# paplorinc/jtokkit

Measured on AMD Instinct MI355X. Metric: input MB/s encoded (cl100k_base), HBM-resident input and output, bit-exact vs CPU oracle, higher is better.
Workload: dtype int32; 1 GPU; cl100k_base, 1M mixed UTF-8 docs (emoji + CJK, ~4 KB each); docs=1000000, bytes=4099377688, docs_per_gpu=1000000, bytes_per_gpu=4099377688, encode=encode() incl. the special-token check

## Files before the change

jtokkit_amd/csrc/jtk_abi.cpp:

```cpp
#include <hip/hip_runtime.h>

#include <algorithm>
#include <cstdio>
#include <cstdlib>
#include <cstring>
#include <new>
#include <string>
#include <vector>
#include <thread>
#include <chrono>

#include "../../include/jtokkit_amd.h"
#include "jtk_chunk_rules.h"
#include "jtk_chunk_prefer_rules.h"
#include "jtk_compact_rules.h"
#include "jtk_decode_rows_rules.h"
#include "jtk_kernels.h"
#include "jtk_maxtok_rules.h"
#include "jtk_tables.h"

namespace {

thread_local std::string g_err;

// ... 198 lines not shown
    if (sp.empty() || n_bytes <= 0) return;
    bool first[256] = {false};
    for (auto& x : sp) if (!x.first.empty()) first[(uint8_t)x.first[0]] = true;
    const size_t slice = (size_t)1 << 22;
    const size_t n_slices = ((size_t)n_bytes + slice - 1) / slice;
    host_slices(n_slices, [&](int, size_t lo, size_t hi) {
        const int64_t b0 = (int64_t)(lo * slice), b1 = std::min<int64_t>(n_bytes, (int64_t)(hi * slice));
        for (int fb = 0; fb < 256; fb++) {
            if (!first[fb]) continue;
            const uint8_t* p = utf8 + b0;
            const uint8_t* const endp = utf8 + b1;
            while (p < endp) {
                p = (const uint8_t*)memchr(p, fb, (size_t)(endp - p));
                if (!p) break;
                const int64_t pos = p - utf8;
                for (auto& x : sp) {
                    const std::string& lit = x.first;
                    if (lit.empty() || (uint8_t)lit[0] != (uint8_t)fb || pos + (int64_t)lit.size() > n_bytes) continue;
                    if (memcmp(p, lit.data(), lit.size()) != 0) continue;
                    const int64_t d = (std::upper_bound(doc_off, doc_off + n_docs + 1, pos) - doc_off) - 1;
                    if (d >= 0 && d < n_docs && pos + (int64_t)lit.size() <= doc_off[d + 1]) flag[(size_t)d] = 1;
                }
                p++;
            }
        }
    });
}



extern "C" {

const char* jtk_version(void) { return "jtokkit_amd 0.1 (gfx950; Unicode " JTK_UNICODE_VERSION " class tables)"; }
const char* jtk_last_error(void) { return g_err.c_str(); }

int jtk_device_count(void) {
    int n = 0;
    hipError_t e = hipGetDeviceCount(&n);
    if (e != hipSuccess) return fail(JTK_ERR_NO_DEVICE, std::string("hipGetDeviceCount: ") + hipGetErrorString(e));
    return n;
}

int jtk_encoding_create(const char* name, int pattern_kind, const uint8_t* tiktoken, size_t tiktoken_len,
                        const char* const* special_literals, const int32_t* special_ids, int n_specials,
                        int device, jtk_encoding** out) {
    if (!out) return fail(JTK_ERR_INVALID_ARGUMENT, "out is NULL");
    *out = nullptr;
    if (!tiktoken || n_specials < 0 || (n_specials > 0 && (!special_literals || !special_ids)))
        return fail(JTK_ERR_INVALID_ARGUMENT, "bad arguments");
    if (n_specials > JTK_MAX_SPECIALS) return fail(JTK_ERR_INVALID_ARGUMENT, "too many special tokens");
    for (int i = 0; i < n_specials; i++) {
        const size_t l = strlen(special_literals[i]);
        if (l < 1 || l > JTK_SPECIAL_MAXLEN)
            return fail(JTK_ERR_INVALID_ARGUMENT, "special-token literals must be 1..65535 bytes long");
        if (special_ids[i] < 0 || special_ids[i] > JTK_MAX_SPECIAL_ID)
            return fail(JTK_ERR_INVALID_ARGUMENT, "special-token id out of range");
    }
    jtk_encoding* enc = new (std::nothrow) jtk_encoding();
    if (!enc) return fail(JTK_ERR_OUT_OF_MEMORY, "out of host memory");
    std::string err;
    int rc = jtk_build_tables(name, pattern_kind, tiktoken, tiktoken_len, special_literals, special_ids, n_specials,
                              enc->host, err);
    if (rc != JTK_OK) { delete enc; return fail(rc, err); }
    enc->tok_len.assign((size_t)enc->host.max_id + 1 + (size_t)enc->host.n_missing, 1);
    {
        int64_t top = (int64_t)enc->host.max_id + (int64_t)enc->host.n_missing;
        for (auto& sp : enc->host.specials) top = std::max<int64_t>(top, sp.second);
        enc->hb = jtk_compact_hb(top);
    }
    for (size_t i = 0; i <= (size_t)enc->host.max_id; i++) enc->tok_len[i] = (uint32_t)enc->host.id_to_bytes[i].size();

    int ndev = 0;
    if (hipGetDeviceCount(&ndev) != hipSuccess || ndev <= 0) {
        delete enc;
        return fail(JTK_ERR_NO_DEVICE, "no HIP device: jtokkit_amd has no CPU path");
    }
    if (device < 0 || device >= ndev) { delete enc; return fail(JTK_ERR_INVALID_ARGUMENT, "device index out of range"); }
    enc->device = device;
    auto cleanup = [&]() { enc->uc1.release(); enc->uc2.release(); enc->uclds.release(); enc->splittab.release(); enc->brank.release(); enc->pairs.release(); enc->tok8.release(); enc->tok16.release(); enc->bprank.release(); enc->bpbits.release(); enc->bpcum.release(); enc->bpranks.release(); enc->pairin.release(); enc->dec_off.release(); enc->dec_blob.release(); enc->longtok.release(); enc->longblob.release(); enc->specials.release(); enc->bnd.release(); delete enc; };
#define ENC_TRY(expr) do { hipError_t e_ = (expr); if (e_ != hipSuccess) { cleanup(); return fail(JTK_ERR_HIP, std::string(#expr) + ": " + hipGetErrorString(e_)); } } while (0)
    ENC_TRY(hipSetDevice(device));
    const size_t tok8_bytes = (enc->host.tok8.size() * sizeof(JtkTok8Slot) + 31) & ~(size_t)31;
    std::vector<uint8_t> uc_image;
    if (sizeof(jtk_uc_stage1_init) <= JTK_UC_LDS_STAGE1 && JTK_UC_LDS_STAGE1 + sizeof(jtk_uc_stage2_init) <= (size_t)JTK_UC_LDS_UNITS * 16) {
        uc_image.assign((size_t)JTK_UC_LDS_UNITS * 16, 0);
        memcpy(uc_image.data(), jtk_uc_stage1_init, sizeof(jtk_uc_stage1_init));
        memcpy(uc_image.data() + JTK_UC_LDS_STAGE1, jtk_uc_stage2_init, sizeof(jtk_uc_stage2_init));
    }
    if (enc->uc1.ensure(sizeof(jtk_uc_stage1_init)) || enc->uc2.ensure(sizeof(jtk_uc_stage2_init)) ||
        enc->uclds.ensure(uc_image.size() + 16) || enc->splittab.ensure(256 * sizeof(JtkCode4)) ||
        enc->brank.ensure(256 * 4) || enc->pairs.ensure(enc->host.pair_buckets.size() * sizeof(JtkPairBucket)) ||
        enc->tok8.ensure(tok8_bytes + enc->host.tok16.size() * sizeof(JtkTok16Slot) + 32) ||
        enc->bprank.ensure(65536 * 4) ||
        enc->bpbits.ensure(1024 * 8) || enc->bpcum.ensure(1024 * 2) || enc->bpranks.ensure(JTK_BP_MAX * 4) || enc->pairin.ensure(2048 * 4)) { cleanup(); return JTK_ERR_OUT_OF_MEMORY; }
    ENC_TRY(hipMemcpy(enc->uc1.p, jtk_uc_stage1_init, sizeof(jtk_uc_stage1_init), hipMemcpyHostToDevice));
    ENC_TRY(hipMemcpy(enc->uc2.p, jtk_uc_stage2_init, sizeof(jtk_uc_stage2_init), hipMemcpyHostToDevice));
    if (!uc_image.empty()) ENC_TRY(hipMemcpy(enc->uclds.p, uc_image.data(), uc_image.size(), hipMemcpyHostToDevice));
    ENC_TRY(hipMemcpy(enc->brank.p, enc->host.byte_rank, 256 * 4, hipMemcpyHostToDevice));
    ENC_TRY(hipMemcpy(enc->pairs.p, enc->host.pair_buckets.data(), enc->host.pair_buckets.size() * sizeof(JtkPairBucket), hipMemcpyHostToDevice));
    ENC_TRY(hipMemcpy(enc->tok8.p, enc->host.tok8.data(), enc->host.tok8.size() * sizeof(JtkTok8Slot), hipMemcpyHostToDevice));
    ENC_TRY(hipMemcpy((uint8_t*)enc->tok8.p + tok8_bytes, enc->host.tok16.data(), enc->host.tok16.size() * sizeof(JtkTok16Slot), hipMemcpyHostToDevice));
    ENC_TRY(hipMemcpy(enc->bprank.p, enc->host.bp_rank.data(), 65536 * 4, hipMemcpyHostToDevice));
    ENC_TRY(hipMemcpy(enc->bpbits.p, enc->host.bp_bits.data(), 1024 * 8, hipMemcpyHostToDevice));
    ENC_TRY(hipMemcpy(enc->bpcum.p, enc->host.bp_cum.data(), 1024 * 2, hipMemcpyHostToDevice));
    ENC_TRY(hipMemcpy(enc->bpranks.p, enc->host.bp_ranks.data(), JTK_BP_MAX * 4, hipMemcpyHostToDevice));
    ENC_TRY(hipMemcpy(enc->pairin.p, enc->host.pair_in_token.data(), 2048 * 4, hipMemcpyHostToDevice));
    {
        uint32_t n_ids = enc->host.max_id + 1;
        for (auto& sp : enc->host.specials) if (sp.second >= 0 && (uint32_t)sp.second + 1 > n_ids) n_ids = (uint32_t)sp.second + 1;
        std::vector<const std::string*> str(n_ids, nullptr);
        for (uint32_t i = 0; i <= enc->host.max_id; i++) if (enc->host.id_present[i]) str[i] = &enc->host.id_to_bytes[i];
        for (auto& sp : enc->host.specials) if (sp.second >= 0 && !str[(size_t)sp.second]) str[(size_t)sp.second] = &sp.first;
        std::vector<uint32_t> off(n_ids + 1, 0);
        std::string blob;
        for (uint32_t i = 0; i < n_ids; i++) { off[i] = (uint32_t)blob.size(); if (str[i]) blob += *str[i]; }
        off[n_ids] = (uint32_t)blob.size();
        blob.append(16, '\0');
        if (enc->dec_off.ensure(off.size() * 4) || enc->dec_blob.ensure(blob.size())) { cleanup(); return JTK_ERR_OUT_OF_MEMORY; }
        ENC_TRY(hipMemcpy(enc->dec_off.p, off.data(), off.size() * 4, hipMemcpyHostToDevice));
        ENC_TRY(hipMemcpy(enc->dec_blob.p, blob.data(), blob.size(), hipMemcpyHostToDevice));
        enc->n_ids_table = n_ids;
        std::vector<uint32_t> bits((n_ids + 31) / 32 + 1, 0);
        for (uint32_t i = 0; i < n_ids; i++)
            if (!str[i] || str[i]->empty() || ((uint8_t)(*str[i])[0] & 0xC0) != 0x80) bits[i >> 5] |= 1u << (i & 31);
        if (enc->bnd.ensure(bits.size() * 4)) { cleanup(); return JTK_ERR_OUT_OF_MEMORY; }
        ENC_TRY(hipMemcpy(enc->bnd.p, bits.data(), bits.size() * 4, hipMemcpyHostToDevice));
    }
    if (!enc->host.long_tok.empty()) {
        if (enc->longtok.ensure(enc->host.long_tok.size() * sizeof(JtkLongTokSlot)) || enc->longblob.ensure(enc->host.long_blob.size())) { cleanup(); return JTK_ERR_OUT_OF_MEMORY; }
        ENC_TRY(hipMemcpy(enc->longtok.p, enc->host.long_tok.data(), enc->host.long_tok.size() * sizeof(JtkLongTokSlot), hipMemcpyHostToDevice));
        ENC_TRY(hipMemcpy(enc->longblob.p, enc->host.long_blob.data(), enc->host.long_blob.size(), hipMemcpyHostToDevice));
    }
    JtkDeviceTables& dt = enc->dt;
    memset(&dt, 0, sizeof(dt));
    dt.longtok.slots = (const JtkLongTokSlot*)enc->longtok.p;
    dt.longtok.blob = (const uint8_t*)enc->longblob.p;
    dt.longtok.n = (uint32_t)enc->host.long_tok.size();
    dt.longtok.max_len = enc->host.long_max_len;
    dt.uc.stage1 = (const uint8_t*)enc->uc1.p;
    dt.uc.stage2 = (const uint32_t*)enc->uc2.p;
    dt.uc_lds_image = uc_image.empty() ? nullptr : (const uint32_t*)enc->uclds.p;
    dt.split_tab = (const uint32_t*)enc->splittab.p;
    dt.byte_rank = (const uint32_t*)enc->brank.p;
    dt.pairs.buckets = (const JtkPairBucket*)enc->pairs.p;
    dt.pairs.bits = enc->host.pair_bits;
    dt.tok8.slots = (const JtkTok8Slot*)enc->tok8.p;
    dt.tok8.bits = enc->host.tok8_bits;
    dt.tok16.slots = (const JtkTok16Slot*)((const uint8_t*)enc->tok8.p + tok8_bytes);
    dt.tok16.n = enc->host.tok16_n;
    dt.bp_rank = (const uint32_t*)enc->bprank.p;
    dt.bp.bits = (const uint64_t*)enc->bpbits.p;
    dt.bp.cum = (const uint16_t*)enc->bpcum.p;
    dt.bp.ranks = (const uint32_t*)enc->bpranks.p;
    dt.pair_in_token = (const uint32_t*)enc->pairin.p;
    dt.kind = pattern_kind;
    dt.pseudo_base = enc->host.n_missing ? enc->host.pseudo_base : 0u;
    dt.n_specials = n_specials;
    {
        std::vector<uint32_t> off((size_t)n_specials + 1, 0);
        std::vector<uint8_t> blob;
        for (int i = 0; i < n_specials; i++) {
            const size_t l = strlen(special_literals[i]);
            blob.insert(blob.end(), (const uint8_t*)special_literals[i], (const uint8_t*)special_literals[i] + l);
            off[(size_t)i + 1] = (uint32_t)blob.size();
            const uint8_t f = (uint8_t)special_literals[i][0];
            dt.special_first[f >> 5] |= 1u << (f & 31);
        }
        const size_t off_bytes = align_up(off.size() * 4, 16);
        if (enc->specials.ensure(off_bytes + blob.size() + 16)) { cleanup(); return JTK_ERR_OUT_OF_MEMORY; }
        ENC_TRY(hipMemcpy(enc->specials.p, off.data(), off.size() * 4, hipMemcpyHostToDevice));
// ... 2103 lines not shown
```

jtokkit_amd/csrc/jtk_block_classify.h:

```cpp
#ifndef JTK_BLOCK_CLASSIFY_H
#define JTK_BLOCK_CLASSIFY_H

#include "jtk_common.h"
#include "jtk_split_masks.h"

enum : uint32_t {
    JTK_F_L = 1u << 0, JTK_F_N = 1u << 1, JTK_F_W = 1u << 2, JTK_F_NL = 1u << 3, JTK_F_SP = 1u << 4, JTK_F_AP = 1u << 5,
    JTK_F_CONT = 1u << 6, JTK_F_LEAD = 1u << 7,
    JTK_F_S1 = 1u << 8, JTK_F_RV = 1u << 9, JTK_F_E = 1u << 10, JTK_F_LL = 1u << 11, JTK_F_C5 = 1u << 12, JTK_F_BF = 1u << 13,
    JTK_F_LT = 1u << 14,
    JTK_F_ULL = 1u << 15
};

JTK_HD uint32_t jtk_byte_code(uint32_t b, bool case_insensitive) {
    uint32_t c = 0;
    if (b < 0x80u) {
        const uint32_t cls = jtk_class_of_ascii(b);
        if (cls == JTK_CLS_L) c |= JTK_F_L;
        if (cls == JTK_CLS_N) c |= JTK_F_N;
        if (cls == JTK_CLS_W) c |= JTK_F_W;
        if (b == '\r' || b == '\n') c |= JTK_F_NL;
        if (b == 0x20u) c |= JTK_F_SP;
        if (b == '\'') c |= JTK_F_AP;
        const uint32_t f = (case_insensitive && (b - 'A') < 26u) ? (b | 0x20u) : b;
        if (f == 's' || f == 't' || f == 'm' || f == 'd') c |= JTK_F_S1;
        if (f == 'r' || f == 'v') c |= JTK_F_RV;
        if (f == 'e') c |= JTK_F_E;
        if (f == 'l') c |= JTK_F_LL;
    } else {
        if ((b & 0xC0u) == 0x80u) c |= JTK_F_CONT; else c |= JTK_F_LEAD;
        if (b == 0xC5u) c |= JTK_F_C5;
        if (b == 0xBFu) c |= JTK_F_BF;
    }
    return c;
}

struct JtkCode4 { uint32_t x, y, z, w; };
JTK_HD JtkCode4 jtk_code4(uint32_t code) {
    JtkCode4 e;
    e.x = (code & 1u) | ((code >> 1) & 1u) << 8 | ((code >> 2) & 1u) << 16 | ((code >> 3) & 1u) << 24;
    e.y = ((code >> 4) & 1u) | ((code >> 5) & 1u) << 8 | ((code >> 6) & 1u) << 16 | ((code >> 7) & 1u) << 24;
    e.z = ((code >> 8) & 1u) | ((code >> 9) & 1u) << 8 | ((code >> 10) & 1u) << 16 | ((code >> 11) & 1u) << 24;
    e.w = ((code >> 12) & 1u) | ((code >> 13) & 1u) << 8 | ((code >> 14) & 1u) << 16 | ((code >> 15) & 1u) << 24;
    return e;
}

JTK_HD uint32_t jtk_shl1_or(uint32_t a, uint32_t e) {
#if defined(__HIP_DEVICE_COMPILE__)
    uint32_t r;
    asm("v_lshl_or_b32 %0, %1, 1, %2" : "=v"(r) : "v"(a), "v"(e));
    return r;
#else
    return (a << 1) | e;
#endif
}

JTK_HD uint32_t jtk_byteperm(uint32_t hi, uint32_t lo, uint32_t sel) {
#if defined(__HIP_DEVICE_COMPILE__)
    return __builtin_amdgcn_perm(hi, lo, sel);
#else
    const uint64_t v = ((uint64_t)hi << 32) | lo;
    uint32_t r = 0;
    for (int q = 0; q < 4; q++) r |= (uint32_t)((v >> (8 * ((sel >> (8 * q)) & 7u))) & 255u) << (8 * q);
    return r;
#endif
}

JTK_HD void jtk_transpose4x4_bytes(uint32_t g0, uint32_t g1, uint32_t g2, uint32_t g3, uint32_t (&o)[4]) {
    const uint32_t t0 = jtk_byteperm(g1, g0, 0x05010400u), t1 = jtk_byteperm(g3, g2, 0x05010400u);
    const uint32_t t2 = jtk_byteperm(g1, g0, 0x07030602u), t3 = jtk_byteperm(g3, g2, 0x07030602u);
    o[0] = jtk_byteperm(t1, t0, 0x05040100u); o[1] = jtk_byteperm(t1, t0, 0x07060302u);
    o[2] = jtk_byteperm(t3, t2, 0x05040100u); o[3] = jtk_byteperm(t3, t2, 0x07060302u);
}

template <class Tab4>
JTK_HD void jtk_block_masks_ascii(const uint32_t (&d)[16], const Tab4& tab, JtkBlk& k, uint64_t& lead_out, uint64_t& lt_out,
                                  uint64_t& ull_out) {
    uint32_t a[8][4];
#pragma unroll
    for (int g = 0; g < 8; g++) {
        uint32_t a0, a1, a2, a3;
        {
            const JtkCode4 e = tab[d[2 * g + 1] >> 24];
            a0 = e.x; a1 = e.y; a2 = e.z; a3 = e.w;
        }
#pragma unroll
        for (int q = 6; q >= 0; q--) {
            const uint32_t b = (d[2 * g + (q >> 2)] >> (8 * (q & 3))) & 255u;
            const JtkCode4 e = tab[b];
            a0 = jtk_shl1_or(a0, e.x); a1 = jtk_shl1_or(a1, e.y); a2 = jtk_shl1_or(a2, e.z); a3 = jtk_shl1_or(a3, e.w);
        }
        a[g][0] = a0; a[g][1] = a1; a[g][2] = a2; a[g][3] = a3;
    }
    uint64_t m[16];
#pragma unroll
    for (int wd = 0; wd < 4; wd++) {
        uint32_t lo[4], hi[4];
        jtk_transpose4x4_bytes(a[0][wd], a[1][wd], a[2][wd], a[3][wd], lo);
        jtk_transpose4x4_bytes(a[4][wd], a[5][wd], a[6][wd], a[7][wd], hi);
#pragma unroll
        for (int q = 0; q < 4; q++) m[4 * wd + q] = ((uint64_t)hi[q] << 32) | lo[q];
    }
    k.L = m[0]; k.N = m[1]; k.W = m[2]; k.NL = m[3]; k.SP = m[4]; k.AP = m[5]; k.CONT = m[6];
    lead_out = m[7];
    k.S1 = m[8]; k.RV = m[9]; k.E = m[10]; k.LL = m[11]; k.C5 = m[12]; k.BF = m[13];
    lt_out = m[14];
    ull_out = m[15];
}

inline bool jtk_lead_all_letters(const JtkUcTables& uc, uint32_t b) {
    uint32_t lo, hi;
    if (b >= 0xC2u && b <= 0xDFu) { lo = (b & 0x1Fu) << 6; hi = lo + 63u; }
    else if (b == 0xE0u) { lo = 0x800u; hi = 0xFFFu; }
    else if (b == 0xEDu) { lo = 0xD000u; hi = 0xD7FFu; }
    else if (b >= 0xE1u && b <= 0xEFu) { lo = (b & 0x0Fu) << 12; hi = lo + 0xFFFu; }
    else if (b == 0xF0u) { lo = 0x10000u; hi = 0x3FFFFu; }
    else if (b >= 0xF1u && b <= 0xF3u) { lo = (b & 7u) << 18; hi = lo + 0x3FFFFu; }
    else if (b == 0xF4u) { lo = 0x100000u; hi = 0x10FFFFu; }
    else return false;
    for (uint32_t cp = lo; cp <= hi; cp++) if (jtk_class_of_cp(uc, cp) != JTK_CLS_L) return false;
    return true;
}

JTK_HD uint64_t jtk_with_cont_bytes(uint64_t x, uint64_t cont) {
    const uint64_t c1 = (x << 1) & cont, c2 = (c1 << 1) & cont, c3 = (c2 << 1) & cont;
    return x | c1 | c2 | c3;
}

inline void jtk_build_code4_table(bool case_insensitive, const uint32_t (&special_first)[8], const uint32_t (&lead_letters)[8],
                                  JtkCode4 (&out)[256]) {
    for (uint32_t b = 0; b < 256; b++) {
        uint32_t code = jtk_byte_code(b, case_insensitive);
        if ((special_first[b >> 5] >> (b & 31)) & 1u) code |= JTK_F_LT;
        if ((lead_letters[b >> 5] >> (b & 31)) & 1u) code |= JTK_F_ULL;
        out[b] = jtk_code4(code);
    }
}

JTK_HD uint32_t jtk_decode_lead_word(uint32_t w) {
    const uint32_t b0 = w & 255u;
#if defined(__HIP_DEVICE_COMPILE__)
    uint32_t n = (uint32_t)__clz((int)~(b0 << 24));
#else
    uint32_t n = (uint32_t)__builtin_clz(~(b0 << 24));
#endif
    n = n > 4u ? 4u : n;
    const uint32_t t = (b0 << 18) | ((w >> 8) & 0x3Fu) << 12 | ((w >> 16) & 0x3Fu) << 6 | ((w >> 24) & 0x3Fu);
    return (t >> (24u - 6u * n)) & ((2u << (5u * n)) - 1u);
}

template <class Txt4>
JTK_HD void jtk_block_fix_nonascii(const Txt4& txt, const JtkUcTables& uc, uint64_t lead, uint64_t ull, JtkBlk& k,
                                   uint32_t& spill_cls) {
    uint64_t c0 = ull & lead, c1 = 0;
    for (uint64_t m = lead & ~ull; m;) {
        const int ja = jtk_ctz64(m);
        m &= m - 1;
        const int jb = m ? jtk_ctz64(m) : ja;
        m &= m - 1;
        const uint32_t wa = txt.word(ja), wb = txt.word(jb);
        const uint32_t cpa = jtk_decode_lead_word(wa), cpb = jtk_decode_lead_word(wb);
        const uint32_t ca = cpa < 0x10FFFFu ? cpa : 0x10FFFFu, cb = cpb < 0x10FFFFu ? cpb : 0x10FFFFu;
        const uint32_t blka = uc.stage1[ca >> 8], blkb = uc.stage1[cb >> 8];
        const uint32_t wda = uc.stage2[blka * 16 + ((ca & 255u) >> 4)], wdb = uc.stage2[blkb * 16 + ((cb & 255u) >> 4)];
        const uint32_t clsa = (wda >> (2 * (ca & 15u))) & 3u, clsb = (wdb >> (2 * (cb & 15u))) & 3u;
        c0 |= ((uint64_t)(clsa & 1u) << ja) | ((uint64_t)(clsb & 1u) << jb);
        c1 |= ((uint64_t)(clsa >> 1) << ja) | ((uint64_t)(clsb >> 1) << jb);
    }
    spill_cls = JTK_CLS_O;
    if (lead) {
        const int jt = 63 - jtk_clz64(lead);
        if (((~k.CONT >> jt) >> 1) == 0) spill_cls = (uint32_t)((c0 >> jt) & 1ull) | (uint32_t)((c1 >> jt) & 1ull) << 1;
    }
    c0 = jtk_with_cont_bytes(c0, k.CONT);
    c1 = jtk_with_cont_bytes(c1, k.CONT);
    k.L |= c0 & ~c1;
    k.N |= c1 & ~c0;
    k.W |= c0 & c1;
}

JTK_HD void jtk_block_apply_spill(JtkBlk& k, uint32_t prev_spill_cls) {
    const uint64_t c = k.CONT;
    uint64_t head = c & 1ull;
    head |= (head << 1) & c;
    head |= (head << 1) & c;
    if (prev_spill_cls == JTK_CLS_L) k.L |= head;
    else if (prev_spill_cls == JTK_CLS_N) k.N |= head;
    else if (prev_spill_cls == JTK_CLS_W) k.W |= head;
}

#endif
```

jtokkit_amd/csrc/jtk_kernels.h:

```cpp
#ifndef JTK_KERNELS_H
#define JTK_KERNELS_H

#include <hip/hip_runtime.h>
#include <stdint.h>

#include "jtk_common.h"
#include "jtk_pack_rules.h"
#include "jtk_label_rules.h"
#include "jtk_stage_rules.h"
#include "jtk_decode_rows_rules.h"
#include "jtk_charpos_rules.h"
#include "jtk_utf16_rules.h"
#include "jtk_stop_rules.h"

#define JTK_SPLIT_TILE 4096
#define JTK_SPLIT_HALO 64
#define JTK_TILE 2048
#define JTK_QE_POS_MASK ((1ull << 37) - 1ull)
#define JTK_QE_LEN_SHIFT 37
#define JTK_QE_DONE (1ull << 63)
#define JTK_NBINS 7
#define JTK_BIN_TINY 7
#define JTK_TINY_CAP (JTK_TILE / 2)
#define JTK_Q_SHARDS 64
#define JTK_QC_STRIDE 32
#define JTK_QC(bin, shard) (((bin) * JTK_Q_SHARDS + (shard)) * JTK_QC_STRIDE)
#define JTK_BIN_CAP0 (JTK_TILE / 4)
#define JTK_BIN_CAP1 (JTK_TILE / 8)
#define JTK_BIN_CAP2 160
#define JTK_BIN_CAP3 (JTK_TILE / 16)
#define JTK_BIN_CAP4 (JTK_TILE / 32)
#define JTK_BIN_CAP5 (JTK_TILE / 64)
#define JTK_BIN_CAP6 (JTK_TILE / 128)
#define JTK_NBINS_BYTES 3
#define JTK_NBINS_LEAN 5
#define JTK_BIN_MAXLEN 256
#define JTK_M_WGS_PER_SHARD 4
#define JTK_MID_CAP 512
#define JTK_LONG_CAP 8192
#define JTK_GIANT_CAP (1 << 20)
#define JTK_GIANT_CHUNK 256
#define JTK_MAX_SPECIALS 65536
#define JTK_SPECIAL_MAXLEN 65535

#define JTK_UC_LDS_UNITS 768
#define JTK_UC_LDS_STAGE1 4352

struct JtkDeviceTables {
    JtkUcTables uc;
    const uint32_t* uc_lds_image;
    const uint32_t* split_tab;
    const uint32_t* byte_rank;
    JtkPairTable pairs;
    JtkTok8Table tok8;
    JtkTok16Table tok16;
    const uint32_t* bp_rank;
    JtkBpLds bp;
    const uint32_t* pair_in_token;
    JtkLongTokTable longtok;
    int kind;
    uint32_t pseudo_base;
    int n_specials;
    uint32_t special_first[8];
    const uint8_t* special_blob;
    const uint32_t* special_off;
};

#define JTK_PL_HARD 0x80000000u
#define JTK_PL_NOQUEUE 0x40000000u
#define JTK_PL_STAGED 0x20000000u
#define JTK_PL_OFF_SHIFT 17
#define JTK_PL_QI_SHIFT 11
#define JTK_PL_BIN_SHIFT 21
#define JTK_HT_ID_MASK 0x1FFFFu
#define JTK_HT_CNT_SHIFT 17
#define JTK_HT_CNT_MASK 0x3FFFu
#define JTK_HT_ESCAPE 0x3FFFu

struct JtkLongPiece {
    int64_t start;
    int64_t len;
};

struct JtkResult {
    int64_t n_tokens;
    int32_t worst_status;
    uint32_t pad;
};

struct JtkWork {
    const uint8_t* text;
    const int64_t* doc_off;
    int64_t text_base;
    int64_t lead;
    int64_t n_bytes;
    int64_t n_docs;
    int64_t n_words;
    int64_t n_tiles;
    uint32_t count_only;
    uint32_t inline_scan;
    uint32_t check_special;
    uint64_t* docmask;
    uint64_t* piecemask;
    uint64_t* gapmask;
    uint32_t* plist;
    uint32_t* tile_np;
    uint32_t* htok;
    uint32_t* docpre;
    uint32_t* tile_tot;
    int64_t* tile_off;
    uint64_t* qm[JTK_NBINS];
    uint4* qd[JTK_NBINS];
    int64_t q_cap[JTK_NBINS];
    uint64_t* qt;
    int64_t qt_cap;
    uint32_t* q_count;
    uint32_t* q_meta;
    JtkLongPiece* mid_list;
    JtkLongPiece* long_list;
    JtkLongPiece* giant_list;
    uint32_t* mid_count;
    uint32_t* long_count;
    uint32_t* n_giant;
    int32_t* status;
    int32_t* tokens;
    int64_t* tok_off;
    const int64_t* job_tokens;
    int64_t* job_tokens_next;
    int64_t* set_info;
// ... 270 lines not shown
```

jtokkit_amd/csrc/jtk_kernels.hip:

```cpp
#include "jtk_kernels.h"

#include <type_traits>

#include "jtk_device_prims.h"
#include "jtk_merge_core.h"
#include "jtk_merge_order_rules.h"
#include "jtk_block_classify.h"
#include "jtk_split_masks.h"
#include "jtk_split_rules.h"

namespace {

constexpr int WAVE = 64;

__device__ __forceinline__ uint64_t lanemask_lt() {
    const unsigned lane = threadIdx.x & 63u;
    return (1ull << lane) - 1ull;
}

__device__ __forceinline__ void wave_lds_fence() {
    __builtin_amdgcn_fence(__ATOMIC_RELEASE, "wavefront");
    __builtin_amdgcn_wave_barrier();
    __builtin_amdgcn_fence(__ATOMIC_ACQUIRE, "wavefront");
}
// ... 9 lines not shown
}

__global__ void __launch_bounds__(256) k_mark_docs(JtkWork w) {
    const int64_t d = (int64_t)blockIdx.x * blockDim.x + threadIdx.x;
    if (d > w.n_docs) return;
    const int64_t q = w.doc_off[d] - w.text_base;
    const bool bad = q < w.lead || q > w.n_bytes || (d > 0 && w.doc_off[d - 1] - w.text_base > q) || (d == 0 && q != w.lead) ||
                     (d == w.n_docs && q != w.n_bytes);
    if (bad) { atomicMin(&w.result->worst_status, -1 ); return; }
    atomicOr((unsigned long long*)&w.docmask[q >> 6], 1ull << (q & 63));
}

__device__ int64_t find_doc(const JtkWork& w, int64_t p) {
    return jtk_first_gt(w.doc_off, 0, w.n_docs, p + w.text_base) - 1;
}

__device__ void special_check_at(const JtkWork& w, const JtkDeviceTables& t, int64_t p) {
    if (p < 0 || p >= w.n_bytes) return;
    for (int s = 0; s < t.n_specials; s++) {
        const uint32_t o = t.special_off[s];
        const int len = (int)(t.special_off[s + 1] - o);
        if (p + len > w.n_bytes) continue;
        bool eq = true;
        for (int j = 0; j < len && eq; j++) eq = (w.text[p + j] == t.special_blob[o + j]);
        if (!eq) continue;
        const int64_t d = find_doc(w, p);
        if (d >= 0 && p + len <= w.doc_off[d + 1] - w.text_base) atomicMin(&w.status[d], -2 );
    }
}

__global__ void __launch_bounds__(256) k_validate_utf8(JtkWork w) {
    const int64_t p = (int64_t)blockIdx.x * blockDim.x + threadIdx.x;
    if (p >= w.n_bytes) return;
    auto ds = [&](int64_t q) { return q >= w.n_bytes || ((w.docmask[q >> 6] >> (q & 63)) & 1ull) != 0; };
    auto at = [&](int64_t q) -> uint32_t { return (q >= 0 && q < w.n_bytes) ? w.text[q] : 0u; };
    const uint32_t b = w.text[p];
    bool bad = false;
    if (b < 0x80u) return;
    if ((b & 0xC0u) == 0x80u) {
        bad = true;
        int64_t q = p;
        for (int k = 1; k <= 3; k++) {
            if (ds(q)) break;
            q--;
            const uint32_t c = at(q);
            if ((c & 0xC0u) == 0x80u) continue;
            const int len = c >= 0xF0u ? 4 : (c >= 0xE0u ? 3 : (c >= 0xC2u ? 2 : 0));
            bad = !(c >= 0xC2u && c <= 0xF4u && len > k);
            break;
        }
    } else {
        const int len = b >= 0xF0u ? 4 : (b >= 0xE0u ? 3 : 2);
        if (b < 0xC2u || b > 0xF4u) bad = true;
        for (int k = 1; k < len && !bad; k++) {
            const uint32_t c = at(p + k);
            if (ds(p + k) || (c & 0xC0u) != 0x80u) bad = true;
        }
        if (!bad) {
            const uint32_t c1 = at(p + 1);
            if (b == 0xE0u && c1 < 0xA0u) bad = true;
            if (b == 0xEDu && c1 > 0x9Fu) bad = true;
            if (b == 0xF0u && c1 < 0x90u) bad = true;
            if (b == 0xF4u && c1 > 0x8Fu) bad = true;
        }
    }
    if (bad) {
        const int64_t d = find_doc(w, p);
        if (d >= 0) atomicMin(&w.status[d], -6 );
    }
}

struct GlobalText {
    const uint8_t* t; int64_t n;
    __device__ uint32_t byte(int64_t p) const { return (p >= 0 && p < n) ? t[p] : 0u; }
};

constexpr int SPLIT_THREADS = 512;

struct LdsBlockWords {
    const uint32_t* blk; int tid;
    __device__ uint32_t word(int j) const {
        const uint32_t a = (uint32_t)j >> 2;
        const uint32_t lo = blk[a * SPLIT_THREADS + (uint32_t)tid], hi = blk[(a + 1u) * SPLIT_THREADS + (uint32_t)tid];
        return __builtin_amdgcn_alignbyte(hi, lo, (uint32_t)j & 3u);
    }
};
struct GlobalBlockWords {
    const uint8_t* t; int64_t n, p0;
    __device__ uint32_t word(int j) const {
        uint32_t v = 0;
        for (int r = 0; r < 4; r++) { const int64_t p = p0 + j + r; if (p >= 0 && p < n) v |= (uint32_t)t[p] << (8 * r); }
        return v;
    }
};

struct SlowWin {
    typedef int64_t idx_t;
    static constexpr int kMaxWalk = 0;
    const uint8_t* gtext; int64_t n; const uint64_t* docmask; JtkUcTables uc;
    __device__ uint32_t byte(int64_t p) const { return (p >= 0 && p < n) ? gtext[p] : 0u; }
    __device__ uint32_t cb(int64_t p) const {
        if (p >= n || p < 0) return JTK_CB_DS;
        GlobalText g{gtext, n};
        uint32_t c = jtk_class_byte(g, uc, p);
        if ((docmask[p >> 6] >> (p & 63)) & 1ull) c |= JTK_CB_DS;
        return c;
    }
};

constexpr int UC_ROWS = 4;
static_assert(JTK_UC_LDS_UNITS % (64 * UC_ROWS) == 0, "the class table moves in whole groups of rows");
constexpr int SPW = 62;
constexpr int SPLIT_BYTES = (SPLIT_THREADS / 64) * SPW * 64;

__device__ __forceinline__ uint64_t hi_from_prev_lane(uint64_t v) {
    return (uint64_t)(uint32_t)__shfl_up((int)(uint32_t)(v >> 32), 1) << 32;
}
__device__ __forceinline__ uint64_t lo_from_next_lane(uint64_t v) {
    return (uint64_t)(uint32_t)__shfl_down((int)(uint32_t)v, 1);
}

template <int KIND>
__global__ void __launch_bounds__(SPLIT_THREADS) __attribute__((amdgpu_waves_per_eu(4, 4))) k_pretok_split(JtkWork w, JtkDeviceTables t) {
    __shared__ __attribute__((aligned(16))) JtkCode4 s_tab[256];
    __shared__ __attribute__((aligned(16))) uint32_t s_pin[2048];
    __shared__ uint32_t s_blk[17 * SPLIT_THREADS];
    __shared__ uint4 s_uc[JTK_UC_LDS_UNITS];
    __shared__ uint32_t s_uc_ready;
    static_assert(SPLIT_THREADS * 4 == 2048 && SPLIT_THREADS >= 256, "the prologue moves one 16-byte unit per thread");

    const int tid = threadIdx.x, lane = tid & 63, wv = tid >> 6;
    const int64_t B = (int64_t)blockIdx.x * SPLIT_BYTES;
    const int64_t n = w.n_bytes;
    if (tid < 256) reinterpret_cast<uint4*>(s_tab)[tid] = reinterpret_cast<const uint4*>(t.split_tab)[tid];
    reinterpret_cast<uint4*>(s_pin)[tid] = reinterpret_cast<const uint4*>(t.pair_in_token)[tid];
    if (tid == 0) s_uc_ready = 0;
    __syncthreads();

    const int64_t p0 = B - 64 + (int64_t)(wv * SPW + lane) * 64;
    uint32_t d[16];
#pragma unroll
    for (int q = 0; q < 4; q++) {
        const int64_t p = p0 + 16 * q;
        uint4 v = make_uint4(0, 0, 0, 0);
        if (p >= 0 && p + 16 <= n) v = *reinterpret_cast<const uint4*>(w.text + p);
        else if (p >= 0 && p < n) {
            uint32_t tmp[4] = {0, 0, 0, 0};
            for (int r = 0; r < 16; r++) if (p + r < n) tmp[r >> 2] |= (uint32_t)w.text[p + r] << (8 * (r & 3));
            v = make_uint4(tmp[0], tmp[1], tmp[2], tmp[3]);
        }
        d[4 * q] = v.x; d[4 * q + 1] = v.y; d[4 * q + 2] = v.z; d[4 * q + 3] = v.w;
    }
    JtkBlk cu;
    uint64_t lead, lt, ull;
    jtk_block_masks_ascii(d, s_tab, cu, lead, lt, ull);
    if (w.check_special && lane >= 1 && lane <= SPW) {
        for (uint64_t m = lt; m;) {
            const int j = jtk_ctz64(m);
            m &= m - 1;
            special_check_at(w, t, p0 + j);
        }
    }
    {
        uint32_t spill = JTK_CLS_O;
        const bool lds_ok = t.uc_lds_image != nullptr;
        if (__ballot((lead & ~ull) != 0)) {
            if (lds_ok) {
#pragma unroll
                for (int q = 0; q < 16; q++) s_blk[q * SPLIT_THREADS + tid] = d[q];
                s_blk[16 * SPLIT_THREADS + tid] = (uint32_t)__shfl_down((int)d[0], 1);
                if (*(volatile uint32_t*)&s_uc_ready == 0u) {
                    const uint4* src = reinterpret_cast<const uint4*>(t.uc_lds_image);
                    for (uint32_t i0 = 0; i0 < (uint32_t)JTK_UC_LDS_UNITS; i0 += 64 * UC_ROWS) {
                        uint4 v[UC_ROWS];
#pragma unroll
                        for (int q = 0; q < UC_ROWS; q++) v[q] = src[i0 + 64u * q + (uint32_t)lane];
#pragma unroll
                        for (int q = 0; q < UC_ROWS; q++) s_uc[i0 + 64u * q + lane] = v[q];
                    }
                }
                wave_lds_fence();
                if (lane == 0) *(volatile uint32_t*)&s_uc_ready = 1u;
                const LdsBlockWords bw{s_blk, tid};
                const uint8_t* uc_lds = reinterpret_cast<const uint8_t*>(s_uc);
                const JtkUcTables ucl{uc_lds, reinterpret_cast<const uint32_t*>(uc_lds + JTK_UC_LDS_STAGE1)};
                jtk_block_fix_nonascii(bw, ucl, lead, ull, cu, spill);
            } else {
                const GlobalBlockWords bw{w.text, n, p0};
                jtk_block_fix_nonascii(bw, t.uc, lead, ull, cu, spill);
            }
        } else if (__ballot(lead != 0)) {
            struct NoWords { __device__ uint32_t word(int) const { return 0u; } };
            jtk_block_fix_nonascii(NoWords{}, t.uc, lead, ull, cu, spill);
        }
        uint32_t prev_spill = (uint32_t)__shfl_up((int)spill, 1);
        if (lane == 0) prev_spill = JTK_CLS_O;
        jtk_block_apply_spill(cu, prev_spill);
    }
    {
        const int64_t wd = p0 >> 6;
        uint64_t ds = (p0 >= 0 && wd < w.n_words) ? w.docmask[wd] : 0ull;
        if (p0 + 63 >= n) ds |= (p0 >= n) ? ~0ull : ~((1ull << (n - p0)) - 1ull);
        cu.DS = ds;
    }
    uint32_t prev_byte = (uint32_t)__shfl_up((int)(d[15] >> 24), 1);
    if (lane == 0) prev_byte = (p0 > 0 && p0 <= n) ? w.text[p0 - 1] : 0u;

    JtkBlk nx;
    nx.L = nx.N = nx.SP = nx.AP = nx.S1 = nx.RV = nx.C5 = nx.BF = 0;
    nx.W = lo_from_next_lane(cu.W); nx.DS = lo_from_next_lane(cu.DS); nx.CONT = lo_from_next_lane(cu.CONT); nx.NL = lo_from_next_lane(cu.NL);
    nx.E = lo_from_next_lane(cu.E); nx.LL = lo_from_next_lane(cu.LL);
    JtkSplitCarry base;
    base.pL = hi_from_prev_lane(cu.L);   base.pN = hi_from_prev_lane(cu.N);   base.pW = hi_from_prev_lane(cu.W);
    base.pNL = hi_from_prev_lane(cu.NL); base.pSP = hi_from_prev_lane(cu.SP); base.pDS = hi_from_prev_lane(cu.DS);
    base.pCONT = hi_from_prev_lane(cu.CONT);
    base.pS1 = hi_from_prev_lane(cu.S1); base.pRV = hi_from_prev_lane(cu.RV); base.pE = hi_from_prev_lane(cu.E);
    base.pLL = hi_from_prev_lane(cu.LL); base.pC5 = hi_from_prev_lane(cu.C5); base.pBF = hi_from_prev_lane(cu.BF);

    uint64_t oX = 0, oAP = 0, oSW = 0;
    uint32_t oN = 0, oFlags = 0;
    uint64_t ms = 0, slow = 0, nlanes = 0;
    uint32_t ncnt_in = 0;
    bool nunk_in = false;
    for (int round = 0; round < 66; round++) {
        JtkSplitCarry cy = base;
        cy.pX = hi_from_prev_lane(oX);
        cy.pMsAP = hi_from_prev_lane(oAP);
        cy.pSW = hi_from_prev_lane(oSW);
        cy.ncnt = (uint32_t)__shfl_up((int)oN, 1);
        const uint32_t fl = (uint32_t)__shfl_up((int)oFlags, 1);
        cy.n_unknown = (fl & 1u) != 0;
        cy.sw_unknown = (fl & 2u) != 0;
        if (lane == 0) { cy.pX = cy.pMsAP = cy.pSW = 0; cy.ncnt = 0; cy.n_unknown = true; cy.sw_unknown = true; }
        ncnt_in = cy.ncnt;
        nunk_in = cy.n_unknown;
        ms = jtk_split_block<KIND>(cu, nx, cy, slow, nlanes);
        const uint32_t nfl = (cy.n_unknown ? 1u : 0u) | (cy.sw_unknown ? 2u : 0u);
        const bool changed = ((cy.pX ^ oX) >> 61) != 0 || ((cy.pMsAP ^ oAP) >> 61) != 0 || ((cy.pSW ^ oSW) >> 63) != 0
                             || cy.ncnt != oN || nfl != oFlags;
        oX = cy.pX; oAP = cy.pMsAP; oSW = cy.pSW; oN = cy.ncnt; oFlags = nfl;
        if (!__ballot(changed)) break;
    }

    if (KIND == JTK_PAT_CL100K && __ballot(nlanes != 0)) {
        if ((cu.N & cu.CONT) == 0) {
            uint64_t nslow;
            ms |= jtk_split_n_block(cu, base.pN, ncnt_in, nunk_in, nslow);
            slow |= nslow;
            nlanes = 0;
        }
        for (uint64_t m = nlanes; m;) {
            const int j = jtk_ctz64(m);
            m &= m - 1;
            bool s2 = false;
            const bool v = jtk_split_n_lane(cu, ncnt_in, nunk_in, j, s2);
            if (s2) slow |= 1ull << j;
            else if (v) ms |= 1ull << j;
        }
    }
    for (uint64_t m = slow; m;) {
        const int j = jtk_ctz64(m);
        m &= m - 1;
        const SlowWin sw{w.text, n, w.docmask, t.uc};
        bool dummy = false;
        const bool v = jtk_is_piece_start_t<KIND>(sw, p0 + j, dummy);
        ms = v ? (ms | (1ull << j)) : (ms & ~(1ull << j));
    }

    uint64_t cut = 0;
    if ((lead | cu.CONT) != 0 || __popcll(ms) < 6) {
        uint32_t dd[16];
        const uint8_t* text_again = w.text;
        asm volatile("" : "+s"(text_again));
#pragma unroll
        for (int q = 0; q < 4; q++) {
            const int64_t p = p0 + 16 * q;
            uint4 v = make_uint4(0, 0, 0, 0);
            if (p >= 0 && p + 16 <= n) v = *reinterpret_cast<const uint4*>(text_again + p);
            else if (p >= 0 && p < n) {
                uint32_t tmp[4] = {0, 0, 0, 0};
                for (int r = 0; r < 16; r++) if (p + r < n) tmp[r >> 2] |= (uint32_t)w.text[p + r] << (8 * (r & 3));
                v = make_uint4(tmp[0], tmp[1], tmp[2], tmp[3]);
            }
            dd[4 * q] = v.x; dd[4 * q + 1] = v.y; dd[4 * q + 2] = v.z; dd[4 * q + 3] = v.w;
        }
        uint32_t acc[2] = {0u, 0u};
#pragma unroll
        for (int j = 0; j < 64; j++) {
            const int q = j >> 2, r = j & 3;
            const uint32_t hi = dd[q], lo = (j >= 4) ? dd[q - 1] : (prev_byte << 24);
            const uint32_t sel = 0x0C0C0000u | (uint32_t)(r ? (4 + r - 1) : 3) << 8 | (uint32_t)(4 + r);
            const uint32_t pi = __builtin_amdgcn_perm(hi, lo, sel);
            const uint32_t in = s_pin[pi >> 5] >> (pi & 31u);
            acc[j >> 5] = __builtin_amdgcn_alignbit(in, acc[j >> 5], 1);
        }
        cut = ~(((uint64_t)acc[1] << 32) | acc[0]);
    }

    if (lane >= 1 && lane <= SPW) {
        uint64_t valid = 0;
        if (p0 + 63 <= n) valid = ~0ull;
        else if (p0 <= n) valid = (2ull << (n - p0)) - 1ull;
        const int64_t wd = p0 >> 6;
        if (wd < w.n_words) w.piecemask[wd] = (ms | cut) & valid;
    }
}

constexpr int T = JTK_TILE;
constexpr int TW = T / 64;
static_assert(TW <= 64, "tile scans assume at most 64 mask words");
static_assert((T & (T - 1)) == 0, "piece_resolve wraps positions into the tile with a mask");

__host__ __device__ __forceinline__ constexpr int q_off(int bin) {
    return bin == 0 ? 0 : bin == 1 ? JTK_BIN_CAP0 : bin == 2 ? JTK_BIN_CAP0 + JTK_BIN_CAP1 : bin == 3 ? JTK_BIN_CAP0 + JTK_BIN_CAP1 + JTK_BIN_CAP2
         : bin == 4 ? JTK_BIN_CAP0 + JTK_BIN_CAP1 + JTK_BIN_CAP2 + JTK_BIN_CAP3
         : bin == 5 ? JTK_BIN_CAP0 + JTK_BIN_CAP1 + JTK_BIN_CAP2 + JTK_BIN_CAP3 + JTK_BIN_CAP4
         : bin == 6 ? JTK_BIN_CAP0 + JTK_BIN_CAP1 + JTK_BIN_CAP2 + JTK_BIN_CAP3 + JTK_BIN_CAP4 + JTK_BIN_CAP5
         : JTK_BIN_CAP0 + JTK_BIN_CAP1 + JTK_BIN_CAP2 + JTK_BIN_CAP3 + JTK_BIN_CAP4 + JTK_BIN_CAP5 + JTK_BIN_CAP6;
}
constexpr int Q_TOTAL = q_off(JTK_BIN_TINY) + JTK_TINY_CAP;
// ... 1599 lines not shown
```

Measured before the change: 154,900 MB/s.

## Replace codepoint-keyed Unicode class tables in LDS with a byte-keyed compressed image

Builds on the host a new LDS image that maps UTF-8 lead bytes directly to deduplicated class bit-rows, with a second-level index only for 4-byte sequences. The device then classifies non-ASCII characters without decoding code points, and the LDS footprint shrinks from 768 to 640 units. A wave ballot skips the second-level lookup when no lane holds a 4-byte lead. It also drops the unknown-flag tracking in the convergence loop for non-cl100k patterns. The cost is a more complex host-side build that can fail and fall back to the global-memory path, plus an unaligned 64-bit LDS read per lookup.

```diff
diff --git a/jtokkit_amd/csrc/jtk_abi.cpp b/jtokkit_amd/csrc/jtk_abi.cpp
--- a/jtokkit_amd/csrc/jtk_abi.cpp
+++ b/jtokkit_amd/csrc/jtk_abi.cpp
@@ -304,10 +304,11 @@
     ENC_TRY(hipSetDevice(device));
     const size_t tok8_bytes = (enc->host.tok8.size() * sizeof(JtkTok8Slot) + 31) & ~(size_t)31;
     std::vector<uint8_t> uc_image;
-    if (sizeof(jtk_uc_stage1_init) <= JTK_UC_LDS_STAGE1 && JTK_UC_LDS_STAGE1 + sizeof(jtk_uc_stage2_init) <= (size_t)JTK_UC_LDS_UNITS * 16) {
-        uc_image.assign((size_t)JTK_UC_LDS_UNITS * 16, 0);
-        memcpy(uc_image.data(), jtk_uc_stage1_init, sizeof(jtk_uc_stage1_init));
-        memcpy(uc_image.data() + JTK_UC_LDS_STAGE1, jtk_uc_stage2_init, sizeof(jtk_uc_stage2_init));
+    {
+        static_assert(JTK_UCB_BYTES == JTK_UC_LDS_UNITS * 16, "the image fills the LDS copy");
+        const JtkUcTables host_uc{jtk_uc_stage1_init, jtk_uc_stage2_init};
+        uc_image.resize(JTK_UCB_BYTES);
+        if (!jtk_build_uc_bytes_image(host_uc, uc_image.data())) uc_image.clear();
     }
     if (enc->uc1.ensure(sizeof(jtk_uc_stage1_init)) || enc->uc2.ensure(sizeof(jtk_uc_stage2_init)) ||
         enc->uclds.ensure(uc_image.size() + 16) || enc->splittab.ensure(256 * sizeof(JtkCode4)) ||
diff --git a/jtokkit_amd/csrc/jtk_block_classify.h b/jtokkit_amd/csrc/jtk_block_classify.h
--- a/jtokkit_amd/csrc/jtk_block_classify.h
+++ b/jtokkit_amd/csrc/jtk_block_classify.h
@@ -1,5 +1,8 @@
 #ifndef JTK_BLOCK_CLASSIFY_H
 #define JTK_BLOCK_CLASSIFY_H
+
+#include <string.h>
+#include <vector>
 
 #include "jtk_common.h"
 #include "jtk_split_masks.h"
@@ -149,6 +152,19 @@
     return (t >> (24u - 6u * n)) & ((2u << (5u * n)) - 1u);
 }
 
+JTK_HD void jtk_block_place_classes(uint64_t lead, uint64_t c0, uint64_t c1, JtkBlk& k, uint32_t& spill_cls) {
+    spill_cls = JTK_CLS_O;
+    if (lead) {
+        const int jt = 63 - jtk_clz64(lead);
+        if (((~k.CONT >> jt) >> 1) == 0) spill_cls = (uint32_t)((c0 >> jt) & 1ull) | (uint32_t)((c1 >> jt) & 1ull) << 1;
+    }
+    c0 = jtk_with_cont_bytes(c0, k.CONT);
+    c1 = jtk_with_cont_bytes(c1, k.CONT);
+    k.L |= c0 & ~c1;
+    k.N |= c1 & ~c0;
+    k.W |= c0 & c1;
+}
+
 template <class Txt4>
 JTK_HD void jtk_block_fix_nonascii(const Txt4& txt, const JtkUcTables& uc, uint64_t lead, uint64_t ull, JtkBlk& k,
                                    uint32_t& spill_cls) {
@@ -167,16 +183,116 @@
         c0 |= ((uint64_t)(clsa & 1u) << ja) | ((uint64_t)(clsb & 1u) << jb);
         c1 |= ((uint64_t)(clsa >> 1) << ja) | ((uint64_t)(clsb >> 1) << jb);
     }
-    spill_cls = JTK_CLS_O;
-    if (lead) {
-        const int jt = 63 - jtk_clz64(lead);
-        if (((~k.CONT >> jt) >> 1) == 0) spill_cls = (uint32_t)((c0 >> jt) & 1ull) | (uint32_t)((c1 >> jt) & 1ull) << 1;
-    }
-    c0 = jtk_with_cont_bytes(c0, k.CONT);
-    c1 = jtk_with_cont_bytes(c1, k.CONT);
-    k.L |= c0 & ~c1;
-    k.N |= c1 & ~c0;
-    k.W |= c0 & c1;
+    jtk_block_place_classes(lead, c0, c1, k, spill_cls);
+}
+
+#define JTK_UCB_IDX_BLK0 64
+#define JTK_UCB_IDX_CAP 20
+#define JTK_UCB_ROWS_OFF (64 * (JTK_UCB_IDX_BLK0 + JTK_UCB_IDX_CAP))
+#define JTK_UCB_ROWS_CAP 304
+#define JTK_UCB_SMP_ROW0 (JTK_UCB_ROWS_CAP - 256)
+#define JTK_UCB_BYTES (JTK_UCB_ROWS_OFF + 16 * JTK_UCB_ROWS_CAP)
+
+JTK_HD uint32_t jtk_ucb_l1_index(uint32_t w) { return ((w & 63u) << 6) | ((w >> 8) & 63u); }
+JTK_HD bool jtk_ucb_is4(uint32_t w) { return (w & 0x30u) == 0x30u; }
+JTK_HD uint32_t jtk_ucb_idx_offset(uint32_t w, uint32_t e1) { return jtk_ucb_is4(w) ? e1 * 64u + ((w >> 16) & 63u) : 0u; }
+JTK_HD uint32_t jtk_ucb_row4(uint32_t w, uint32_t e2) { return 16u * (e2 + ((w & 0x3007u) == 0u ? 0u : (uint32_t)JTK_UCB_SMP_ROW0)); }
+JTK_HD uint32_t jtk_ucb_class_in_row(const uint8_t* img, uint32_t row, uint32_t w) {
+    const uint32_t sel = w >> 16;
+    const uint64_t p = *reinterpret_cast<const uint64_t*>(img + JTK_UCB_ROWS_OFF + (row | ((sel >> 2) & 8u)));
+    return (((uint32_t)p >> (sel & 31u)) & 1u) | (((uint32_t)(p >> 32) >> (sel & 31u)) & 1u) << 1;
+}
+
+JTK_HD uint32_t jtk_ucb_class_of_word(const uint8_t* img, uint32_t w) {
+    const uint32_t e1 = img[jtk_ucb_l1_index(w)];
+    if (!jtk_ucb_is4(w)) return jtk_ucb_class_in_row(img, 16u * e1, w);
+    return jtk_ucb_class_in_row(img, jtk_ucb_row4(w, img[jtk_ucb_idx_offset(w, e1)]), w >> 8);
+}
+
+template <class Txt4, class Any>
+JTK_HD void jtk_block_fix_nonascii_bytes(const Txt4& txt, const uint8_t* img, uint64_t lead, uint64_t ull, JtkBlk& k,
+                                         uint32_t& spill_cls, const Any& any4) {
+    uint64_t c0 = ull & lead, c1 = 0;
+    for (uint64_t m = lead & ~ull; m;) {
+        const int ja = jtk_ctz64(m);
+        m &= m - 1;
+        const int jb = m ? jtk_ctz64(m) : ja;
+        m &= m - 1;
+        uint32_t wa = txt.word(ja), wb = txt.word(jb);
+        const uint32_t e1a = img[jtk_ucb_l1_index(wa)], e1b = img[jtk_ucb_l1_index(wb)];
+        const bool fa = jtk_ucb_is4(wa), fb = jtk_ucb_is4(wb);
+        uint32_t rowa = 16u * e1a, rowb = 16u * e1b;
+        if (any4(fa || fb)) {
+            const uint32_t e2a = img[jtk_ucb_idx_offset(wa, e1a)], e2b = img[jtk_ucb_idx_offset(wb, e1b)];
+            if (fa) { rowa = jtk_ucb_row4(wa, e2a); wa >>= 8; }
+            if (fb) { rowb = jtk_ucb_row4(wb, e2b); wb >>= 8; }
+        }
+        const uint32_t clsa = jtk_ucb_class_in_row(img, rowa, wa), clsb = jtk_ucb_class_in_row(img, rowb, wb);
+        c0 |= ((uint64_t)(clsa & 1u) << ja) | ((uint64_t)(clsb & 1u) << jb);
+        c1 |= ((uint64_t)(clsa >> 1) << ja) | ((uint64_t)(clsb >> 1) << jb);
+    }
+    jtk_block_place_classes(lead, c0, c1, k, spill_cls);
+}
+
+inline bool jtk_build_uc_bytes_image(const JtkUcTables& uc, uint8_t* out) {
+    struct Row { uint32_t b[4]; };
+    auto row_of = [&](uint32_t w, int vary) {
+        Row r;
+        memset(r.b, 0, 16);
+        for (uint32_t v = 0; v < 64; v++) {
+            const uint32_t cp = jtk_decode_lead_word(w | v << (8 * vary));
+            const uint32_t cls = jtk_class_of_cp(uc, cp < 0x10FFFFu ? cp : 0x10FFFFu);
+            r.b[2 * (v >> 5)] |= (cls & 1u) << (v & 31);
+            r.b[2 * (v >> 5) + 1] |= (cls >> 1) << (v & 31);
+        }
+        return r;
+    };
+    std::vector<Row> pool;
+    std::vector<uint8_t> used;
+    auto intern = [&](const Row& r, uint8_t by) {
+        for (size_t i = 0; i < pool.size(); i++) if (!memcmp(pool[i].b, r.b, 16)) { used[i] |= by; return (uint32_t)i; }
+        pool.push_back(r);
+        used.push_back(by);
+        return (uint32_t)(pool.size() - 1);
+    };
+    std::vector<uint32_t> l1(4096), idx;
+    for (uint32_t b0 = 0xC0u; b0 < 0xF0u; b0++)
+        for (uint32_t b1 = 0; b1 < 64; b1++) l1[jtk_ucb_l1_index(b0 | b1 << 8)] = intern(row_of(b0 | b1 << 8, 2), 1);
+    for (uint32_t b0 = 0xF0u; b0 <= 0xFFu; b0++)
+        for (uint32_t b1 = 0; b1 < 64; b1++) {
+            uint32_t blk[64];
+            for (uint32_t b2 = 0; b2 < 64; b2++) blk[b2] = intern(row_of(b0 | b1 << 8 | b2 << 16, 3), 0);
+            uint32_t e1 = 0x30u;
+            if (((b0 | b1 << 8) & 0x3007u) == 0u)
+                for (e1 = 0; e1 < 0x30u && memcmp(&l1[e1 * 64], blk, sizeof(blk)); ) e1++;
+            if (e1 == 0x30u) {
+                size_t at = 0;
+                while (at < idx.size() && memcmp(&idx[at], blk, sizeof(blk))) at += 64;
+                if (at == idx.size()) {
+                    idx.insert(idx.end(), blk, blk + 64);
+                    for (uint32_t b2 = 0; b2 < 64; b2++) used[blk[b2]] |= 2;
+                }
+                e1 = JTK_UCB_IDX_BLK0 + (uint32_t)(at / 64);
+            }
+            l1[jtk_ucb_l1_index(b0 | b1 << 8)] = e1;
+        }
+    std::vector<uint32_t> number(pool.size());
+    uint32_t next = 0;
+    for (uint8_t group : {1, 3, 2}) {
+        if (group == 3 && next < JTK_UCB_SMP_ROW0) next = JTK_UCB_SMP_ROW0;
+        for (size_t i = 0; i < pool.size(); i++) if (used[i] == group) number[i] = next++;
+        if (group == 3 && next > 256u) return false;
+    }
+    if (next > JTK_UCB_ROWS_CAP || idx.size() > 64u * JTK_UCB_IDX_CAP) return false;
+    memset(out, 0, JTK_UCB_BYTES);
+    for (uint32_t b0 = 0xC0u; b0 <= 0xFFu; b0++)
+        for (uint32_t b1 = 0; b1 < 64; b1++) {
+            const uint32_t i = jtk_ucb_l1_index(b0 | b1 << 8);
+            out[i] = (uint8_t)(b0 < 0xF0u ? number[l1[i]] : l1[i]);
+        }
+    for (size_t i = 0; i < idx.size(); i++) out[64 * JTK_UCB_IDX_BLK0 + i] = (uint8_t)(number[idx[i]] - JTK_UCB_SMP_ROW0);
+    for (size_t i = 0; i < pool.size(); i++) memcpy(out + JTK_UCB_ROWS_OFF + 16 * number[i], pool[i].b, 16);
+    return true;
 }
 
 JTK_HD void jtk_block_apply_spill(JtkBlk& k, uint32_t prev_spill_cls) {
diff --git a/jtokkit_amd/csrc/jtk_kernels.h b/jtokkit_amd/csrc/jtk_kernels.h
--- a/jtokkit_amd/csrc/jtk_kernels.h
+++ b/jtokkit_amd/csrc/jtk_kernels.h
@@ -43,8 +43,7 @@
 #define JTK_MAX_SPECIALS 65536
 #define JTK_SPECIAL_MAXLEN 65535
 
-#define JTK_UC_LDS_UNITS 768
-#define JTK_UC_LDS_STAGE1 4352
+#define JTK_UC_LDS_UNITS 640
 
 struct JtkDeviceTables {
     JtkUcTables uc;
diff --git a/jtokkit_amd/csrc/jtk_kernels.hip b/jtokkit_amd/csrc/jtk_kernels.hip
--- a/jtokkit_amd/csrc/jtk_kernels.hip
+++ b/jtokkit_amd/csrc/jtk_kernels.hip
@@ -115,7 +115,7 @@
     __device__ uint32_t word(int j) const {
         const uint32_t a = (uint32_t)j >> 2;
         const uint32_t lo = blk[a * SPLIT_THREADS + (uint32_t)tid], hi = blk[(a + 1u) * SPLIT_THREADS + (uint32_t)tid];
-        return __builtin_amdgcn_alignbyte(hi, lo, (uint32_t)j & 3u);
+        return __builtin_amdgcn_alignbyte(hi, lo, (uint32_t)j);
     }
 };
 struct GlobalBlockWords {
@@ -141,8 +141,9 @@
     }
 };
 
-constexpr int UC_ROWS = 4;
+constexpr int UC_ROWS = 5;
 static_assert(JTK_UC_LDS_UNITS % (64 * UC_ROWS) == 0, "the class table moves in whole groups of rows");
+static_assert(JTK_UC_LDS_UNITS * 16 == JTK_UCB_BYTES, "the LDS copy holds the byte-keyed image of jtk_block_classify.h");
 constexpr int SPW = 62;
 constexpr int SPLIT_BYTES = (SPLIT_THREADS / 64) * SPW * 64;
 
@@ -215,9 +216,8 @@
                 wave_lds_fence();
                 if (lane == 0) *(volatile uint32_t*)&s_uc_ready = 1u;
                 const LdsBlockWords bw{s_blk, tid};
-                const uint8_t* uc_lds = reinterpret_cast<const uint8_t*>(s_uc);
-                const JtkUcTables ucl{uc_lds, reinterpret_cast<const uint32_t*>(uc_lds + JTK_UC_LDS_STAGE1)};
-                jtk_block_fix_nonascii(bw, ucl, lead, ull, cu, spill);
+                jtk_block_fix_nonascii_bytes(bw, reinterpret_cast<const uint8_t*>(s_uc), lead, ull, cu, spill,
+                                             [](bool four) { return __ballot(four) != 0; });
             } else {
                 const GlobalBlockWords bw{w.text, n, p0};
                 jtk_block_fix_nonascii(bw, t.uc, lead, ull, cu, spill);
@@ -268,7 +268,7 @@
         ncnt_in = cy.ncnt;
         nunk_in = cy.n_unknown;
         ms = jtk_split_block<KIND>(cu, nx, cy, slow, nlanes);
-        const uint32_t nfl = (cy.n_unknown ? 1u : 0u) | (cy.sw_unknown ? 2u : 0u);
+        const uint32_t nfl = KIND == JTK_PAT_CL100K ? (cy.n_unknown ? 1u : 0u) | (cy.sw_unknown ? 2u : 0u) : 0u;
         const bool changed = ((cy.pX ^ oX) >> 61) != 0 || ((cy.pMsAP ^ oAP) >> 61) != 0 || ((cy.pSW ^ oSW) >> 63) != 0
                              || cy.ncnt != oN || nfl != oFlags;
         oX = cy.pX; oAP = cy.pMsAP; oSW = cy.pSW; oN = cy.ncnt; oFlags = nfl;
```

New measurement: 156,800 MB/s (median of 6 runs). 1.2% higher.
